# uwoseis/zephyr

Hardware: NVIDIA B200
Metric: source-frequency wavefields/sec (higher is better)
Workload: dtype c128

## Files before the change

### zephyr_b200/csrc/hz_api.cu

```cuda
#include <algorithm>
#include <cmath>
#include <cstdio>
#include <cstring>
#include <new>
#include <string>
#include <type_traits>
#include <vector>

#include "hz_platform.h"
#include "hz_assemble.cuh"
#include "hz_gemm.cuh"
#include "hz_factor.cuh"
#include "hz_factor_f32.cuh"
#include "hz_c64.cuh"
#include "hz_tf32.cuh"
#include "hz_solve.cuh"
#include "hz_survey.cuh"
#include "../../include/zephyr_b200.h"

constexpr int PROF_EVERY = 16, PROF_MAX = 4096;

struct hz_ctx {
    int device = 0, dtype = 0, disc = 0, nf = 1;
    int nx = 0, nz = 0, b = 0, nPML = 10;
// ... 4 lines not shown
    cudaStream_t stream = nullptr, stream2 = nullptr;
    cudaStream_t stream1 = nullptr;
    cudaEvent_t ev_fork = nullptr, ev_join = nullptr, ev_join0 = nullptr;
    cplx* c = nullptr;
    double *rho = nullptr, *theta = nullptr, *eps = nullptr, *delta = nullptr;
    cplx* coef = nullptr;
    cplx* Kp = nullptr;
    double* binv = nullptr;
    cplx* pmltab = nullptr;
    bool have_model = false, assembled = false, factored = false;
    cplx* Sinv = nullptr;
    cplxf* Sinv64 = nullptr;
    cplxf* Scratch64[2] = {nullptr, nullptr};
    cplxf *Rf[2] = {nullptr, nullptr}, *Cf[2] = {nullptr, nullptr}, *Pgf[2] = {nullptr, nullptr};
    int c64_tf32 = 1;
    int tf32_sms = 0;
    bool tf32_active = false;
    int ldb64 = 0;
    i64 y_S = -1;
#ifndef HZ_EMU
    alignas(64) CUtensorMap mapA;
    alignas(64) CUtensorMap mapY[2];
#endif
    int c64_fp64_factor = 1;
    cplx* Ring[2][2] = {{nullptr, nullptr}, {nullptr, nullptr}};
    i64 mid = -1;
    int store_every = 1;
    int store_used = 1;
    i64 nslots = 0;
    cplx *Rbuf[2] = {nullptr, nullptr}, *Cbuf[2] = {nullptr, nullptr};
    cplx* Pg[2] = {nullptr, nullptr};
    int* d_flag = nullptr;
    int gj_seq = 0;
    int gj_service = 2;
    int gj_colper = 1;
    int gj_coltile = 0;
    int service_fallbacks = 0;
    bool svc_on[2] = {false, false};
    cudaStream_t svc_stream[2] = {nullptr, nullptr};
    cudaEvent_t ev_svc[2] = {nullptr, nullptr};
    GjJob* d_mail = nullptr;
    GjBlockJob* d_mail2 = nullptr;
    cplx* d_Tg = nullptr;
    int* d_cflag = nullptr;
    int* d_mail_flag = nullptr;
    unsigned long long* d_done = nullptr;
    unsigned long long done_total[2] = {0, 0};
    int seq_chain[2] = {0, 0};
    cplx* Scratch[2] = {nullptr, nullptr};
    int* d_sync[2] = {nullptr, nullptr};
    size_t sync_bytes = 0;
    int gj_lean = 0;
    int gemm_3m = 1;
    int gj_colpair = 0;
    int gj_colslow = 0;
    int gj_crit = 1;
    int gj_pdl = 0;
    int gj_order = 0;
    int gj_inv = -1;
    int gj_tile = 3;
    int gj_trace = 0;
    long long* d_trace[2] = {nullptr, nullptr};
    bool trace_now = false;
    int trace_chain = 0;
    int trace_steps = 0, trace_grid = 0;
    int factor_graph = 0;
#ifndef HZ_EMU
    cudaGraphExec_t fgraph = nullptr;
#endif
    unsigned long long fgraph_key = 0, fgraph_seen = 0, fgraph_want = 0;
    long long fgraph_launches = 0;
    int fgraph_replays = 0;
    unsigned opt_epoch = 0;
    cudaEvent_t ev_svc_join[2] = {nullptr, nullptr};
    cudaEvent_t ev_fork2 = nullptr;
    int gj_mode = 1;
    cplx* Ybuf[2] = {nullptr, nullptr};
    i64 ycap = 0;
    cplx *Qsave = nullptr, *Rres = nullptr;
    i64 qcap = 0;
    int probe_check = 1;
    double probe_limit = 0.0;
    bool probe_pending = false;
    cplx* Qprobe = nullptr;
    double last_probe = -1.0;
    int* d_err = nullptr;
    double* d_norm = nullptr;
    bool prof_on = false;
    long long prof_tick[2] = {0, 0};
    std::vector<cudaEvent_t> prof_ev[2];
    long long prof_launches[2] = {0, 0};
    std::string err;
};

static void prof_begin(hz_ctx* h, int kind, cudaStream_t st, bool& armed) {
    armed = false;
    if (!h->prof_on) return;
    ++h->prof_launches[kind];
    if ((h->prof_tick[kind]++ % PROF_EVERY) != 0 || (int)h->prof_ev[kind].size() >= 2 * PROF_MAX) return;
    cudaEvent_t e0, e1;
    if (cudaEventCreate(&e0) != cudaSuccess) return;
    if (cudaEventCreate(&e1) != cudaSuccess) { cudaEventDestroy(e0); return; }
    h->prof_ev[kind].push_back(e0);
    h->prof_ev[kind].push_back(e1);
    cudaEventRecord(e0, st);
    armed = true;
// ... 757 lines not shown
    } else {
        if ((rc = launch_schur<cplx>(h, i, Xa, Xb, slot, st))) return rc;
        rc = launch_invert_v1(h, slot, chain, st);
    }
    if (rc) return rc;
    if (h->dtype == HZ_C64) {
#ifndef HZ_EMU
        if (h->tf32_active)
            HZ_LAUNCH_EW(convert_planar_kernel, dim3(blocks_for(nb2, 256)), dim3(256), 0, st, (const cplx*)slot, (float*)block64(h, i), h->b, h->ldb64);
        else
#endif
        HZ_LAUNCH_EW(convert_c64_kernel, dim3(blocks_for(nb2, 256)), dim3(256), 0, st, (const cplx*)slot, block64(h, i), nb2);
        HZ_CHECK_LAUNCH(h);
    }
    return HZ_OK;
}

static bool pair_mode(const hz_ctx* h) {
    return h->gj_mode == 4 && !(h->dtype == HZ_C64 && !h->c64_fp64_factor) && !h->gj_trace && h->gj_tile == 3 && h->gj_service != 1 && !h->gj_pdl &&
           !h->gj_coltile && h->gj_colper <= 1 && !h->gj_order && h->gj_inv < 0;
}
static int factor_pair(hz_ctx* h, i64 i0, i64 ia0, i64 ib0, int chain0, i64 i1, i64 ia1, i64 ib1, int chain1, cudaStream_t st) {
    const i64 nb2 = (i64)h->b * h->b;
    int rc;
    cplx* slot[2] = {nullptr, nullptr};
    const i64 ii[2] = {i0, i1}, ia[2] = {ia0, ia1}, ib[2] = {ib0, ib1};
    const int ch[2] = {chain0, chain1};
    for (int c = 0; c < 2; ++c) {
        if (ii[c] < 0) continue;
        const cplx* Xa = ia[c] >= 0 ? block128(h, ia[c], 0) : nullptr;
        const cplx* Xb = ib[c] >= 0 ? block128(h, ib[c], 1) : nullptr;
        slot[c] = block128(h, ii[c], ch[c]);
        cplx* start = gj_start_buffer(h) ? h->Scratch[ch[c]] : slot[c];
        if ((rc = launch_schur<cplx>(h, ii[c], Xa, Xb, start, st))) return rc;
    }
    if ((rc = launch_invert_pair(h, slot[0], ch[0], slot[1], ch[1], st))) return rc;
    if (h->dtype == HZ_C64)
        for (int c = 0; c < 2; ++c) {
            if (ii[c] < 0) continue;
#ifndef HZ_EMU
            if (h->tf32_active)
                HZ_LAUNCH_EW(convert_planar_kernel, dim3(blocks_for(nb2, 256)), dim3(256), 0, st, (const cplx*)slot[c], (float*)block64(h, ii[c]), h->b, h->ldb64);
            else
#endif
            HZ_LAUNCH_EW(convert_c64_kernel, dim3(blocks_for(nb2, 256)), dim3(256), 0, st, (const cplx*)slot[c], block64(h, ii[c]), nb2);
            HZ_CHECK_LAUNCH(h);
        }
    return HZ_OK;
}

int hz_set_option(hz_handle_t h, const char* key, double value) {
    if (!h || !key) return fail(h, HZ_EINVAL, "hz_set_option: NULL argument");
    if (!strcmp(key, "store_every") && (int)value == h->store_every) return HZ_OK;
    if (strcmp(key, "probe_check") && strcmp(key, "probe_limit") && strcmp(key, "gj_trace_chain") && strcmp(key, "factor_graph")) ++h->opt_epoch;
    if (!strcmp(key, "factor_graph")) { h->factor_graph = (int)value; return HZ_OK; }
    if (!strcmp(key, "gj_mode")) { h->gj_mode = (int)value; return HZ_OK; }
    if (!strcmp(key, "gj_colslow")) { h->gj_colslow = (int)value; return HZ_OK; }
    if (!strcmp(key, "gj_colpair")) { h->gj_colpair = (int)value; return HZ_OK; }
    if (!strcmp(key, "gj_lean")) { h->gj_lean = (int)value; return HZ_OK; }
    if (!strcmp(key, "gemm_3m")) { h->gemm_3m = (int)value; h->factored = false; return HZ_OK; }
    if (!strcmp(key, "gj_trace")) { h->gj_trace = (int)value; return HZ_OK; }
    if (!strcmp(key, "gj_trace_chain")) { h->trace_chain = (int)value; return HZ_OK; }
    if (!strcmp(key, "gj_crit")) { h->gj_crit = (int)value; return HZ_OK; }
    if (!strcmp(key, "gj_pdl")) { h->gj_pdl = (int)value; return HZ_OK; }
    if (!strcmp(key, "gj_tile")) { h->gj_tile = (int)value; return HZ_OK; }
    if (!strcmp(key, "gj_colper")) { h->gj_colper = (int)value; return HZ_OK; }
    if (!strcmp(key, "gj_coltile")) { h->gj_coltile = (int)value; return HZ_OK; }
    if (!strcmp(key, "gj_service")) { h->gj_service = (int)value; return HZ_OK; }
    if (!strcmp(key, "gj_order")) { h->gj_order = (int)value; return HZ_OK; }
    if (!strcmp(key, "gj_inv")) { h->gj_inv = (int)value; return HZ_OK; }
    if (!strcmp(key, "store_every")) {
        if (value < 1 || value > 64) return fail(h, HZ_EINVAL, "hz_set_option: store_every must be in [1, 64]");
        if ((int)value != h->store_every) h->factored = false;
        h->store_every = (int)value;
        return HZ_OK;
    }
    if (!strcmp(key, "probe_check")) { h->probe_check = (int)value; return HZ_OK; }
    if (!strcmp(key, "probe_limit")) { h->probe_limit = value; return HZ_OK; }
    if (!strcmp(key, "gj_newton")) {
        const int v = (int)value;
#ifdef HZ_EMU
        hz_gj_newton = v;
#else
        HZ_CUDA(h, cudaSetDevice(h->device));
        HZ_CUDA(h, cudaMemcpyToSymbol(hz_gj_newton, &v, sizeof(int)));
#endif
        h->factored = false;
        return HZ_OK;
    }
    if (!strcmp(key, "tf32_sms")) { h->tf32_sms = (int)value; return HZ_OK; }
    if (!strcmp(key, "c64_tf32")) { h->c64_tf32 = (int)value; h->factored = false; return HZ_OK; }
    if (!strcmp(key, "c64_fp64_factor")) { h->c64_fp64_factor = (int)value; h->factored = false; return HZ_OK; }
    return fail(h, HZ_EINVAL, std::string("hz_set_option: unknown key ") + key);
}

#ifndef HZ_EMU
template <class K>
static void preload_kernel(K kfn) {
    cudaFuncAttributes attr;
    cudaFuncGetAttributes(&attr, kfn);
}
template <class TP>
static void preload_panel_kernels() {
    preload_kernel(couple_kernel<TP, 0>); preload_kernel(residual_kernel<TP, 0>); preload_kernel(gather_col_kernel<TP>);
    preload_kernel(residual_col_kernel<TP, 0>); preload_kernel(norm2_kernel<TP>); preload_kernel(axpy_kernel<TP>);
    preload_kernel(couple_kernel<TP, 1>); preload_kernel(residual_kernel<TP, 1>); preload_kernel(residual_col_kernel<TP, 1>);
    preload_kernel(couple_kernel<TP, 2>); preload_kernel(residual_kernel<TP, 2>); preload_kernel(residual_col_kernel<TP, 2>);
    preload_kernel(finalize_kernel<TP>); preload_kernel(scatter_coo_kernel<TP>); preload_kernel(spmm_csr_kernel<TP>);
    preload_kernel(spmm_percol_kernel<TP>); preload_kernel(spmm_percol_t_kernel<TP>); preload_kernel(gradient_kernel<TP>);
    preload_kernel(misfit_kernel<TP>);
}
static void preload_factor_kernels() {
    static std::atomic<unsigned long long> done{0};
    hz_once_per_device(done, []() {
    for (const GjVariant& v : gj_variants()) {
        preload_kernel(v.fn);
        if (v.fn_lean) preload_kernel(v.fn_lean);
    }
    preload_kernel(gj_block_kernel<4, 2, 2, 4, 1, 2, 1, 2>);
    preload_kernel(gj_pair_kernel<4, 2, 2, 4, 1, 2, 1, 2>);
    preload_kernel(schur_form_kernel<cplx>);
    preload_kernel(schur_form_kernel<cplxf>);
    preload_kernel(convert_c64_kernel); preload_kernel(convert_c128_kernel);
    preload_kernel(convert_planar_kernel); preload_kernel(unconvert_planar_kernel); preload_kernel(couple_planar_kernel);
    preload_kernel(cgemm_tf32_kernel<32>); preload_kernel(cgemm_tf32_kernel<64>); preload_kernel(cgemm_tf32_kernel<128>);
    preload_kernel(cgemm_f32_kernel); preload_kernel(gj_step_f32_kernel); preload_kernel(gj_panel_kernel);
    preload_kernel(gj_step2_kernel<4, 2, 2, 4, 3>);
    preload_kernel(gj_post_quit_kernel);
    preload_kernel(gj_inverter_service);
    preload_kernel(gj_inverter_service2);
    preload_kernel(gj_post_quit2_kernel);
    preload_kernel(node_terms_kernel); preload_kernel(assemble_mz_kernel); preload_kernel(eurus_pml_tables_kernel); preload_kernel(assemble_eurus_kernel);
    preload_kernel(nearest_index_kernel); preload_kernel(kaiser_taps_kernel);
    preload_panel_kernels<cplx>();
    preload_panel_kernels<cplxf>();
    zgemm_for_each_instance<0>([](auto kfn) { preload_kernel(kfn); });
    zgemm_for_each_instance<1>([](auto kfn) { preload_kernel(kfn); });
    zgemm_for_each_instance<2>([](auto kfn) { preload_kernel(kfn); });
    cudaFuncSetAttribute(gj_inverter_service, cudaFuncAttributeMaxDynamicSharedMemorySize, GJ_SERVICE_SMEM);
    cudaFuncSetAttribute(gj_inverter_service2, cudaFuncAttributeMaxDynamicSharedMemorySize, GJ_SERVICE_SMEM);
    cudaGetLastError();
    });
}
#endif

static int factor_attempt(hz_ctx* h, int64_t twist, int* herr_out) {
    if (!h) return fail(h, HZ_EINVAL, "hz_factor: NULL handle");
    if (!h->assembled) return fail(h, HZ_ESTATE, "hz_factor: call hz_assemble first");
    HZ_CUDA(h, cudaSetDevice(h->device));
    const int nz = h->nz, b = h->b;
    i64 mid = twist < 0 ? nz / 2 : twist;
    if (mid >= nz) mid = nz - 1;
    const size_t blk = (size_t)b * b * sizeof(cplx);
    const int kst = h->store_every < 1 ? 1 : h->store_every;
    const i64 nslots = slots_needed(nz, mid, kst);
    if ((h->Sinv || h->Sinv64) && nslots != h->nslots) {
        HZ_CUDA(h, cudaStreamSynchronize(h->stream));
        HZ_CUDA(h, cudaStreamSynchronize(h->stream1));
        HZ_CUDA(h, cudaStreamSynchronize(h->stream2));
        free_dev(h->Sinv);
        free_dev(h->Sinv64);
    }
    bool want_tf32 = false;
// ... 261 lines not shown
    if (herr == 2) return fail(h, HZ_ECUDA, "hz_factor: the pivot-block inverter service did not answer (device-side wait timed out)");
    if (herr) return fail(h, HZ_ESINGULAR, "hz_factor: zero or non-finite pivot in a diagonal block (singular operator or NaN in the model)");
    h->factored = true;
    h->probe_pending = true;
    return HZ_OK;
}

int hz_factor(hz_handle_t h, int64_t twist) {
    int herr = 0;
    int rc = factor_attempt(h, twist, &herr);
    if (rc == HZ_ECUDA && herr == 2 && h && h->gj_service) {
        h->service_fallbacks += 1;
        const int fails = ++g_service_failures;
        const int saved = g_service_unavailable.exchange(1);
        if (fails == 1) fprintf(stderr, "zephyr_b200: pivot-block inverter service did not answer; this factorisation is redone with the in-kernel inverter\n");
        rc = factor_attempt(h, twist, &herr);
        if (fails < 2 && !saved) g_service_unavailable.store(0);
        else if (fails == 2) fprintf(stderr, "zephyr_b200: pivot-block inverter service failed twice in a row; using the in-kernel inverter in this process\n");
    } else if (rc == HZ_OK && h && h->gj_service && !g_service_unavailable.load()) {
        g_service_failures.store(0);
    }
    return rc;
}

int hz_get_block_inverse(hz_handle_t h, int64_t iz, void* out_host) {
    if (!h || !out_host) return fail(h, HZ_EINVAL, "hz_get_block_inverse: NULL argument");
    if (!h->factored) return fail(h, HZ_ESTATE, "hz_get_block_inverse: no factors");
    if (iz < 0 || iz >= h->nz) return fail(h, HZ_EINVAL, "hz_get_block_inverse: iz out of range");
    if (!is_stored(h, iz)) return fail(h, HZ_ESTATE, "hz_get_block_inverse: this block is not kept (store_every > 1); only checkpoints are");
    HZ_CUDA(h, cudaSetDevice(h->device));
    const i64 nb2 = (i64)h->b * h->b;
    if (h->dtype == HZ_C64 && h->tf32_active) {
        std::vector<float> tmp((size_t)2 * h->b * h->ldb64);
        HZ_CUDA(h, cudaMemcpyAsync(tmp.data(), block64(h, iz), tmp.size() * sizeof(float), cudaMemcpyDeviceToHost, h->stream));
        HZ_CUDA(h, cudaStreamSynchronize(h->stream));
        float* o = (float*)out_host;
        const size_t plane = (size_t)h->b * h->ldb64;
        for (int r = 0; r < h->b; ++r)
            for (int c = 0; c < h->b; ++c) {
                o[2 * ((size_t)r * h->b + c)] = tmp[(size_t)r * h->ldb64 + c];
                o[2 * ((size_t)r * h->b + c) + 1] = tmp[plane + (size_t)r * h->ldb64 + c];
            }
        return HZ_OK;
    }
    if (h->dtype == HZ_C64)
        HZ_CUDA(h, cudaMemcpyAsync(out_host, block64(h, iz), (size_t)nb2 * sizeof(cplxf), cudaMemcpyDeviceToHost, h->stream));
    else
        HZ_CUDA(h, cudaMemcpyAsync(out_host, h->Sinv + slot_of(h, iz) * nb2, (size_t)nb2 * sizeof(cplx), cudaMemcpyDeviceToHost, h->stream));
    HZ_CUDA(h, cudaStreamSynchronize(h->stream));
    return HZ_OK;
}

template <class TP>
static int launch_couple(hz_ctx* h, i64 i, TP* X, i64 S, TP* Y, int use_self, double lo, double hi, cudaStream_t st, int zero_self, int op) {
    const int threads = S >= 128 ? 128 : (S >= 64 ? 64 : 32);
    dim3 grid((unsigned)((S + threads - 1) / threads), h->b, 1);
#ifndef HZ_EMU
    if (std::is_same<TP, cplxf>::value && h->tf32_active) {
        const i64 ldk = h->ldb64;
        ++g_hz_launches;
        cudaLaunchConfig_t cfg = {};
        cfg.gridDim = dim3((unsigned)((S + 31) / 32), (unsigned)((h->b + 31) / 32), 1); cfg.blockDim = dim3(256); cfg.dynamicSmemBytes = 0; cfg.stream = st;
        cudaLaunchAttribute at[1];
        at[0].id = cudaLaunchAttributeProgrammaticStreamSerialization;
        at[0].val.programmaticStreamSerializationAllowed = 1;
        cfg.attrs = at; cfg.numAttrs = 1;
        cudaLaunchKernelEx(&cfg, couple_planar_kernel, (const cplx*)h->coef, h->nf, h->nx, h->nz, (int)i, (cplxf*)X, S, (float*)Y, ldk, (i64)S * ldk,
                           use_self, lo, hi, zero_self);
        HZ_CHECK_LAUNCH(h);
        return HZ_OK;
    }
#endif
    auto kfn = op == HZ_OP_T ? couple_kernel<TP, 1> : (op == HZ_OP_H ? couple_kernel<TP, 2> : couple_kernel<TP, 0>);
    HZ_LAUNCH_EW(kfn, grid, dim3(threads), 0, st, (const cplx*)h->coef, h->nf, h->nx, h->nz, (int)i, X, S, Y, use_self, lo, hi);
    HZ_CHECK_LAUNCH(h);
    return HZ_OK;
}

static int launch_block_gemm(hz_ctx* h, i64 i, const cplx* Y, cplx* X, i64 S, double alpha, int beta, cudaStream_t st, int op) {
    GemmParams p;
    p.A = h->Sinv + slot_of(h, i) * (i64)h->b * h->b; p.lda = h->b;
    p.B = Y; p.ldb = S;
    p.C = X + i * (i64)h->nx * S; p.ldc = S;
    p.M = h->b; p.N = (int)S; p.K = h->b;
    p.alpha = alpha; p.beta = beta;
    p.sub_c0 = p.sub_c1 = 0;
    p.row_nx = h->nf > 1 ? h->nx : 0;
    p.row_fs = h->N;
    bool armed;
    prof_begin(h, 0, st, armed);
    const bool m3 = (h->gemm_3m & 1) != 0;
    if (op == HZ_OP_T) zgemm_launch<1>(p, st, h->num_sms, -1, m3);
    else if (op == HZ_OP_H) zgemm_launch<2>(p, st, h->num_sms, -1, m3);
    else zgemm_launch<0>(p, st, h->num_sms, -1, m3);
    prof_end(h, 0, st, armed);
    HZ_CHECK_LAUNCH(h);
    return HZ_OK;
}
static int launch_block_gemm(hz_ctx* h, i64 i, const cplxf* Y, cplxf* X, i64 S, double alpha, int beta, cudaStream_t st, int ) {
#ifndef HZ_EMU
    if (h->tf32_active) {
        Tf32Params tp;
        tp.M = h->b; tp.N = (int)S; tp.K = h->b;
        tp.a_plane0 = (int)(2 * slot_of(h, i));
        tp.y_plane0 = 0;
        tp.C = X + i * (i64)h->nx * S; tp.ldc = S;
        tp.alpha = (float)alpha;
        tp.row_nx = h->nf > 1 ? h->nx : 0;
        tp.row_fs = h->N;
        tp.k_per_split = 0;
        tp.dbg = nullptr; tp.mode = 0; tp.force_split = 0;
        bool armed;
        prof_begin(h, 0, st, armed);
        cgemm_tf32_launch(h->mapA, h->mapY[(const cplx*)Y == h->Ybuf[1] ? 1 : 0], tp, h->tf32_sms > 0 ? h->tf32_sms : h->num_sms, st);
        prof_end(h, 0, st, armed);
        HZ_CHECK_LAUNCH(h);
        return HZ_OK;
    }
#endif
    CGemmParams p;
    p.A = block64(h, i); p.lda = h->b;
    p.B = Y; p.ldb = S;
    p.C = X + i * (i64)h->nx * S; p.ldc = S;
    p.M = h->b; p.N = (int)S; p.K = h->b;
    p.alpha = (float)alpha; p.beta = beta;
    p.row_nx = h->nf > 1 ? h->nx : 0;
    p.row_fs = h->N;
    bool armed;
    prof_begin(h, 0, st, armed);
    cgemm_f32_launch(p, st);
    prof_end(h, 0, st, armed);
    HZ_CHECK_LAUNCH(h);
    return HZ_OK;
}

static int recompute_segment(hz_ctx* h, int chain, i64 j, cudaStream_t st) {
    const int k = h->store_used;
    const i64 len = chain == 0 ? h->mid : (i64)h->nz - 1 - h->mid;
    const i64 p0 = j * k, p1 = std::min<i64>((j + 1) * k - 1, len - 1);
    const i64 nb2 = (i64)h->b * h->b;
    for (i64 p = p0; p < p1; ++p) {
        const i64 i = chain_row(h, chain, p), prev = p > 0 ? chain_row(h, chain, p - 1) : -1;
        if (h->dtype == HZ_C64 && h->c64_fp64_factor && p == p0 && prev >= 0) {
#ifndef HZ_EMU
            if (h->tf32_active)
                HZ_LAUNCH_EW(unconvert_planar_kernel, dim3(blocks_for(nb2, 256)), dim3(256), 0, st, (const float*)block64(h, prev), h->Ring[chain][prev & 1], h->b, h->ldb64);
            else
#endif
            HZ_LAUNCH_EW(convert_c128_kernel, dim3(blocks_for(nb2, 256)), dim3(256), 0, st, (const cplxf*)block64(h, prev), h->Ring[chain][prev & 1], nb2);
            HZ_CHECK_LAUNCH(h);
        }
        const int rc = factor_block(h, i, chain == 0 ? prev : -1, chain == 1 ? prev : -1, chain, st);
        if (rc) return rc;
    }
    return HZ_OK;
}

template <class TP>
static int solve_inplace(hz_ctx* h, TP* X, i64 S, i64 zf, i64 zl, int op) {
    const i64 nz = h->nz, mid = h->mid;
    const int k = h->store_used;
    if (zf < 0 || zf >= nz) zf = 0;
    if (zl < 0 || zl >= nz) zl = nz - 1;
    if (zl < zf) { zf = 0; zl = nz - 1; }
    cudaStream_t st[2] = {h->stream, h->stream2};
    TP* Y[2] = {(TP*)h->Ybuf[0], (TP*)h->Ybuf[1]};
    const i64 len[2] = {mid, nz - 1 - mid};
    int rc;
    HZ_CUDA(h, cudaEventRecord(h->ev_fork, st[0]));
    HZ_CUDA(h, cudaStreamWaitEvent(st[1], h->ev_fork, 0));
    const bool top_fwd = zf < mid, bot_fwd = zl > mid;
    const i64 pfirst[2] = {zf, nz - 1 - zl};
    for (int c = 0; c < 2; ++c) {
        for (i64 p = pfirst[c]; p < len[c]; ++p) {
            if (k > 1 && (p == pfirst[c] || p % k == 0) && (rc = recompute_segment(h, c, p / k, st[c]))) return rc;
            const i64 i = chain_row(h, c, p);
            const double sg = p > pfirst[c] ? -1.0 : 0.0;
            if ((rc = launch_couple<TP>(h, i, X, S, Y[c], 1, c == 0 ? sg : 0.0, c == 0 ? 0.0 : sg, st[c], 1, op))) return rc;
            if ((rc = launch_block_gemm(h, i, (const TP*)Y[c], X, S, 1.0, 0, st[c], op))) return rc;
        }
    }
    HZ_CUDA(h, cudaEventRecord(h->ev_join, st[1]));
    HZ_CUDA(h, cudaStreamWaitEvent(st[0], h->ev_join, 0));
    if ((rc = launch_couple<TP>(h, mid, X, S, Y[0], 1, top_fwd ? -1.0 : 0.0, bot_fwd ? -1.0 : 0.0, st[0], 1, op))) return rc;
    if ((rc = launch_block_gemm(h, mid, (const TP*)Y[0], X, S, 1.0, 0, st[0], op))) return rc;
    HZ_CUDA(h, cudaEventRecord(h->ev_fork, st[0]));
    HZ_CUDA(h, cudaStreamWaitEvent(st[1], h->ev_fork, 0));
    const i64 nmax = len[0] > len[1] ? len[0] : len[1];
    for (i64 t = 1; t <= nmax; ++t) {
        for (int c = 0; c < 2; ++c) {
            if (t > len[c]) continue;
            const i64 p = len[c] - t, i = chain_row(h, c, p);
            if (k > 1 && (t == 1 || p % k == k - 1) && (rc = recompute_segment(h, c, p / k, st[c]))) return rc;
            if ((rc = launch_couple<TP>(h, i, X, S, Y[c], 0, c == 0 ? 0.0 : 1.0, c == 0 ? 1.0 : 0.0, st[c], 0, op))) return rc;
            if ((rc = launch_block_gemm(h, i, (const TP*)Y[c], X, S, -1.0, 1, st[c], op))) return rc;
        }
    }
    HZ_CUDA(h, cudaEventRecord(h->ev_join, st[1]));
    HZ_CUDA(h, cudaStreamWaitEvent(st[0], h->ev_join, 0));
    if (k > 1) {
        int herr = 0;
        HZ_CUDA(h, cudaMemcpyAsync(&herr, h->d_err, sizeof(int), cudaMemcpyDeviceToHost, st[0]));
        HZ_CUDA(h, cudaStreamSynchronize(st[0]));
        if (herr) return fail(h, HZ_ESINGULAR, "hz_solve: zero or non-finite pivot while recomputing block inverses between checkpoints");
    }
    return HZ_OK;
}

template <class TP>
static int launch_residual(hz_ctx* h, const TP* X, const TP* Q, i64 S, TP* R, int op) {
    const int threads = S >= 128 ? 128 : (S >= 64 ? 64 : 32);
    const i64 rows = (i64)h->nf * h->N;
    dim3 grid((unsigned)((S + threads - 1) / threads), (unsigned)(rows < 65535 ? rows : 65535), (unsigned)((rows + 65534) / 65535));
    auto kfn = op == HZ_OP_T ? residual_kernel<TP, 1> : (op == HZ_OP_H ? residual_kernel<TP, 2> : residual_kernel<TP, 0>);
    HZ_LAUNCH_EW(kfn, grid, dim3(threads), 0, h->stream, (const cplx*)h->coef, h->nf, h->nx, h->nz, X, Q, S, R);
    HZ_CHECK_LAUNCH(h);
    return HZ_OK;
}

template <class TP>
static int solve_impl(hz_ctx* h, int op, TP* X, int64_t S, double premul_re, double premul_im, int conjugate,
                      int64_t z_first, int64_t z_last, int refine, double* resid_host) {
    const i64 rows = (i64)h->nf * h->N, n = rows * S;
    if (h->ycap < S) {
        HZ_CUDA(h, cudaStreamSynchronize(h->stream));
        HZ_CUDA(h, cudaStreamSynchronize(h->stream2));
        for (int k = 0; k < 2; ++k) {
            free_dev(h->Ybuf[k]);
            HZ_CUDA(h, cudaMalloc((void**)&h->Ybuf[k], (size_t)h->b * S * sizeof(cplx)));
        }
        h->ycap = S;
        h->y_S = -1;
    }
#ifndef HZ_EMU
    if (std::is_same<TP, cplxf>::value && h->tf32_active && h->y_S != S) {
        for (int k = 0; k < 2; ++k)
            if (!t32_make_map(&h->mapY[k], (const float*)h->Ybuf[k], h->b, S, 2, h->ldb64, T32_KS, t32_tile_n(S), false))
                return fail(h, HZ_ECUDA, "hz_solve: cuTensorMapEncodeTiled failed for the right-hand-side planes");
        h->y_S = S;
    }
#endif
    const bool want_resid = refine > 0 || resid_host != nullptr;
    if (want_resid && h->qcap < S) {
        HZ_CUDA(h, cudaStreamSynchronize(h->stream));
        free_dev(h->Qsave); free_dev(h->Rres);
        HZ_CUDA(h, cudaMalloc((void**)&h->Qsave, (size_t)n * sizeof(TP)));
        HZ_CUDA(h, cudaMalloc((void**)&h->Rres, (size_t)n * sizeof(TP)));
        h->qcap = S;
// ... 367 lines not shown
```

### zephyr_b200/csrc/hz_gemm.cuh

```cuda
#pragma once
#include "hz_platform.h"

struct GemmParams {
    const cplx* A; i64 lda;
    const cplx* B; i64 ldb;
    cplx* C; i64 ldc;
    int M, N, K;
    double alpha;
    int beta;
    int sub_c0, sub_c1;
    int row_nx; i64 row_fs;
};

constexpr int GEMM_KB = 32;
constexpr int GEMM_LDA = GEMM_KB + 4;

template <int MI, int NI, int WM, int WN, int STAGES, int KS = 1>
struct GemmCfg {
    static constexpr int TM = 8 * MI * WM, TN = 8 * NI * WN, THREADS = 32 * WM * WN * KS;
    static constexpr int LDB = TN + 2;
    static constexpr int A_ELEMS = TM * GEMM_LDA, B_ELEMS = GEMM_KB * LDB;
    static constexpr int SMEM = STAGES * (A_ELEMS + B_ELEMS) * (int)sizeof(cplx);
};

template <int MI, int NI, int WM, int WN, int STAGES, int KS = 1, bool M3 = false, int OPA = 0>
__global__ void __launch_bounds__(32 * WM * WN * KS, 1) zgemm_dmma_kernel(GemmParams p) {
    typedef GemmCfg<MI, NI, WM, WN, STAGES, KS> Cfg;
    constexpr int TM = Cfg::TM, TN = Cfg::TN, NT = Cfg::THREADS, LDB = Cfg::LDB;
    constexpr bool AT = OPA != 0, ACONJ = OPA == 2;
    constexpr int LDAT = TM + 2;
    static_assert(OPA >= 0 && OPA <= 2, "op(A) is N, T or C");
    static_assert(!AT || GEMM_KB * LDAT <= Cfg::A_ELEMS, "the k-major A tile must fit the A stage");
    HZ_SMEM(smem_raw);
    cplx* sA = reinterpret_cast<cplx*>(smem_raw);
    cplx* sB = sA + STAGES * Cfg::A_ELEMS;

    const int tid = threadIdx.x;
    const int warp = tid >> 5, lane = tid & 31;
    const int g = lane >> 2, t = lane & 3;
    const int wk = warp / (WM * WN), w2 = warp % (WM * WN);
    const int wm = w2 / WN, wn = w2 % WN;
    const int m0 = blockIdx.y * TM, n0 = blockIdx.x * TN;
    const int KT = (p.K + GEMM_KB - 1) / GEMM_KB;

    static_assert(NT % GEMM_KB == 0 && NT % TN == 0, "staging assumes whole rows per thread stride");
    constexpr int RA = AT ? NT / TM : NT / GEMM_KB, RB = NT / TN;
    constexpr int NA = AT ? (GEMM_KB + RA - 1) / RA : (TM * GEMM_KB + NT - 1) / NT, NBL = (GEMM_KB * TN + NT - 1) / NT;
    const int a_r0 = AT ? tid / TM : tid / GEMM_KB, a_kk = AT ? tid % TM : tid % GEMM_KB;
    const int b_k0 = tid / TN, b_c = tid % TN;
    const cplx* a_base = AT ? p.A + (i64)a_r0 * p.lda + (m0 + a_kk) : p.A + (i64)(m0 + a_r0) * p.lda + a_kk;
    const cplx* b_base = p.B + (i64)b_k0 * p.ldb + (n0 + b_c);
    const i64 a_step = (i64)RA * p.lda, b_step = (i64)RB * p.ldb;
    const bool a_col_ok = AT && a_r0 < RA && m0 + a_kk < p.M;
    const bool b_col_ok = n0 + b_c < p.N;
    auto stage_op = [&](int op, int k0, cplx* a, cplx* b) {
        if (op < NA) {
            const int u = op, r = a_r0 + u * RA;
            if constexpr (AT) {
                if (a_r0 < RA && r < GEMM_KB) {
                    const bool ok = a_col_ok && (k0 + r < p.K);
                    cp_async16(a + r * LDAT + a_kk, ok ? a_base + (i64)k0 * p.lda + u * a_step : p.A, ok);
                }
            } else if (u * NT + tid < TM * GEMM_KB) {
                const bool ok = (m0 + r < p.M) && (k0 + a_kk < p.K);
                cp_async16(a + r * GEMM_LDA + a_kk, ok ? a_base + u * a_step + k0 : p.A, ok);
            }
        } else {
            const int u = op - NA, kk = b_k0 + u * RB;
            if (u * NT + tid < GEMM_KB * TN) {
                const bool ok = b_col_ok && (k0 + kk < p.K);
                cp_async16(b + kk * LDB + b_c, ok ? b_base + (i64)k0 * p.ldb + u * b_step : p.B, ok);
            }
        }
    };
    auto load_stage = [&](int kt, int st) {
#pragma unroll
        for (int op = 0; op < NA + NBL; ++op) stage_op(op, kt * GEMM_KB, sA + st * Cfg::A_ELEMS, sB + st * Cfg::B_ELEMS);
    };

    double cre[MI][NI][2], cim[MI][NI][2];
    double c2[M3 ? MI : 1][M3 ? NI : 1][2];
#pragma unroll
    for (int mi = 0; mi < MI; ++mi)
#pragma unroll
        for (int ni = 0; ni < NI; ++ni) {
            cre[mi][ni][0] = cre[mi][ni][1] = cim[mi][ni][0] = cim[mi][ni][1] = 0.0;
            if constexpr (M3) c2[mi][ni][0] = c2[mi][ni][1] = 0.0;
        }

#pragma unroll
    for (int s = 0; s < STAGES - 1; ++s) {
        if (s < KT) load_stage(s, s);
        cp_async_commit();
    }

    constexpr int S4 = GEMM_KB / 4 / KS;
    constexpr int OPS = (NA + NBL + S4 - 1) / S4;
    for (int kt = 0; kt < KT; ++kt) {
        cp_async_wait<STAGES - 2>();
        __syncthreads();
        const int nk = kt + STAGES - 1;
        const bool refill = nk < KT;
        cplx* na = sA + (nk % STAGES) * Cfg::A_ELEMS;
        cplx* nb = sB + (nk % STAGES) * Cfg::B_ELEMS;
        const cplx* a = AT ? sA + (kt % STAGES) * Cfg::A_ELEMS + t * LDAT + wm * MI * 8 + g
                           : sA + (kt % STAGES) * Cfg::A_ELEMS + (wm * MI * 8 + g) * GEMM_LDA + t;
        const cplx* b = sB + (kt % STAGES) * Cfg::B_ELEMS + t * LDB + wn * NI * 8 + g;
#pragma unroll
        for (int k4s = 0; k4s < S4; ++k4s) {
            const int k4 = k4s * KS + wk;
            cplx af[MI], bf[NI];
#pragma unroll
            for (int mi = 0; mi < MI; ++mi) af[mi] = AT ? a[k4 * 4 * LDAT + mi * 8] : a[mi * 8 * GEMM_LDA + k4 * 4];
#pragma unroll
            for (int ni = 0; ni < NI; ++ni) bf[ni] = b[k4 * 4 * LDB + ni * 8];
            if constexpr (M3) {
                double as[MI], bs[NI];
#pragma unroll
                for (int mi = 0; mi < MI; ++mi) as[mi] = ACONJ ? af[mi].re - af[mi].im : af[mi].re + af[mi].im;
#pragma unroll
                for (int ni = 0; ni < NI; ++ni) bs[ni] = bf[ni].re + bf[ni].im;
#pragma unroll
                for (int mi = 0; mi < MI; ++mi)
#pragma unroll
                    for (int ni = 0; ni < NI; ++ni) {
                        dmma884(cre[mi][ni][0], cre[mi][ni][1], af[mi].re, bf[ni].re);
                        dmma884(c2[mi][ni][0], c2[mi][ni][1], af[mi].im, bf[ni].im);
                    }
                if (refill) {
#pragma unroll
                    for (int op = k4s * OPS; op < (k4s + 1) * OPS && op < NA + NBL; ++op) stage_op(op, nk * GEMM_KB, na, nb);
                }
#pragma unroll
                for (int mi = 0; mi < MI; ++mi)
#pragma unroll
                    for (int ni = 0; ni < NI; ++ni) dmma884(cim[mi][ni][0], cim[mi][ni][1], as[mi], bs[ni]);
            } else {
#pragma unroll
            for (int mi = 0; mi < MI; ++mi)
#pragma unroll
                for (int ni = 0; ni < NI; ++ni) {
                    dmma884(cre[mi][ni][0], cre[mi][ni][1], af[mi].re, bf[ni].re);
                    dmma884(cim[mi][ni][0], cim[mi][ni][1], af[mi].re, bf[ni].im);
                }
            if (refill) {
// ... 34 lines not shown
            for (int mi = 0; mi < MI; ++mi)
#pragma unroll
                for (int ni = 0; ni < NI; ++ni) {
                    red[(mi * NI + ni) * 64] = mk(cre[mi][ni][0], cim[mi][ni][0]);
                    red[(mi * NI + ni) * 64 + 1] = mk(cre[mi][ni][1], cim[mi][ni][1]);
                }
        }
        __syncthreads();
        if (wk > 0) return;
#pragma unroll
        for (int mi = 0; mi < MI; ++mi)
#pragma unroll
            for (int ni = 0; ni < NI; ++ni)
#pragma unroll
                for (int j = 0; j < 2; ++j) {
                    const cplx v = red[(mi * NI + ni) * 64 + j];
                    cre[mi][ni][j] += v.re;
                    cim[mi][ni][j] += v.im;
                }
    }

#pragma unroll
    for (int mi = 0; mi < MI; ++mi) {
        const int r = m0 + (wm * MI + mi) * 8 + g;
        if (r >= p.M) continue;
        const i64 crow = p.row_nx ? (i64)(r / p.row_nx) * p.row_fs + (r % p.row_nx) : (i64)r;
        cplx* crp = p.C + crow * p.ldc;
#pragma unroll
        for (int ni = 0; ni < NI; ++ni) {
#pragma unroll
            for (int j = 0; j < 2; ++j) {
                const int cidx = n0 + (wn * NI + ni) * 8 + 2 * t + j;
                if (cidx >= p.N) continue;
                cplx v = mk(p.alpha * cre[mi][ni][j], p.alpha * cim[mi][ni][j]);
                if (p.beta) {
                    cplx cin;
                    if (cidx >= p.sub_c0 && cidx < p.sub_c1) cin = mk(r == cidx ? 1.0 : 0.0);
                    else cin = crp[cidx];
                    v = v + cin;
                }
                crp[cidx] = v;
            }
        }
    }
}

template <int MI, int NI, int WM, int WN, int STAGES, int KS = 1, bool M3 = false, int OPA = 0>
static inline int zgemm_launch_cfg(const GemmParams& p, cudaStream_t stream) {
    typedef GemmCfg<MI, NI, WM, WN, STAGES, KS> Cfg;
    auto kfn = zgemm_dmma_kernel<MI, NI, WM, WN, STAGES, KS, M3, OPA>;
    static std::atomic<unsigned long long> configured{0};
    hz_once_per_device(configured, [&]() { cudaFuncSetAttribute(kfn, cudaFuncAttributeMaxDynamicSharedMemorySize, Cfg::SMEM); });
    dim3 grid((p.N + Cfg::TN - 1) / Cfg::TN, (p.M + Cfg::TM - 1) / Cfg::TM, 1);
    HZ_LAUNCH_IND(kfn, grid, dim3(Cfg::THREADS), Cfg::SMEM, stream, p);
    return 0;
}

struct GemmTile { int tm, tn; };
static const GemmTile kGemmTiles[] = {{64, 64}, {56, 64}, {48, 64}, {40, 64}, {32, 64}, {32, 32}, {16, 32}};
constexpr int kNumGemmTiles = sizeof(kGemmTiles) / sizeof(kGemmTiles[0]);

static inline int zgemm_pick(int M, int N, int num_sms) {
    double best = -1.0;
    int besti = 0;
    for (int i = 0; i < kNumGemmTiles; ++i) {
        const i64 tiles = (i64)((M + kGemmTiles[i].tm - 1) / kGemmTiles[i].tm) * ((N + kGemmTiles[i].tn - 1) / kGemmTiles[i].tn);
        const i64 waves = (tiles + num_sms - 1) / num_sms;
        double eff = (double)M * N / ((double)waves * num_sms * kGemmTiles[i].tm * kGemmTiles[i].tn);
        eff *= 1.0 + 0.02 * (kGemmTiles[i].tm * kGemmTiles[i].tn) / 4096.0;
        if (eff > best) { best = eff; besti = i; }
    }
    return besti;
}

static inline int zgemm_tile_id(int cand, bool m3) {
    const int which = cand + (m3 ? 16 : 0);
    return which == 17 ? 24 : which;
}

template <int OPA, class F>
static inline void zgemm_for_each_instance(F f) {
    f(zgemm_dmma_kernel<4, 2, 2, 4, 3, 1, false, OPA>); f(zgemm_dmma_kernel<7, 1, 1, 8, 3, 1, false, OPA>);
    f(zgemm_dmma_kernel<6, 1, 1, 8, 3, 1, false, OPA>); f(zgemm_dmma_kernel<5, 1, 1, 8, 3, 1, false, OPA>);
    f(zgemm_dmma_kernel<2, 2, 2, 4, 4, 1, false, OPA>); f(zgemm_dmma_kernel<2, 1, 2, 4, 4, 1, false, OPA>);
    f(zgemm_dmma_kernel<1, 1, 2, 4, 4, 1, false, OPA>);
    f(zgemm_dmma_kernel<4, 2, 2, 4, 3, 1, true, OPA>); f(zgemm_dmma_kernel<6, 1, 1, 8, 3, 1, true, OPA>);
    f(zgemm_dmma_kernel<5, 1, 1, 8, 3, 1, true, OPA>); f(zgemm_dmma_kernel<2, 2, 2, 4, 4, 1, true, OPA>);
    f(zgemm_dmma_kernel<2, 1, 2, 4, 4, 1, true, OPA>); f(zgemm_dmma_kernel<1, 1, 2, 4, 4, 1, true, OPA>);
    f(zgemm_dmma_kernel<7, 2, 1, 4, 3, 2, true, OPA>);
    if constexpr (OPA == 0) {
        f(zgemm_dmma_kernel<7, 1, 1, 8, 3, 2>); f(zgemm_dmma_kernel<4, 2, 2, 4, 3, 2>); f(zgemm_dmma_kernel<6, 1, 1, 8, 3, 2>);
        f(zgemm_dmma_kernel<5, 1, 1, 8, 3, 2>); f(zgemm_dmma_kernel<7, 2, 1, 4, 3>); f(zgemm_dmma_kernel<7, 2, 1, 4, 3, 2>);
        f(zgemm_dmma_kernel<7, 1, 1, 8, 3, 1, true>); f(zgemm_dmma_kernel<7, 2, 1, 4, 3, 1, true>); f(zgemm_dmma_kernel<7, 1, 1, 8, 3, 2, true>);
    }
}

template <int OPA = 0>
static inline int zgemm_launch(const GemmParams& p, cudaStream_t stream, int num_sms, int force_tile = -1, bool m3 = false) {
    const int which = force_tile >= 0 ? force_tile : zgemm_tile_id(zgemm_pick(p.M, p.N, num_sms), m3);
    switch (which) {
        case 16: return zgemm_launch_cfg<4, 2, 2, 4, 3, 1, true, OPA>(p, stream);
        case 18: return zgemm_launch_cfg<6, 1, 1, 8, 3, 1, true, OPA>(p, stream);
        case 19: return zgemm_launch_cfg<5, 1, 1, 8, 3, 1, true, OPA>(p, stream);
        case 20: return zgemm_launch_cfg<2, 2, 2, 4, 4, 1, true, OPA>(p, stream);
        case 21: return zgemm_launch_cfg<2, 1, 2, 4, 4, 1, true, OPA>(p, stream);
        case 22: return zgemm_launch_cfg<1, 1, 2, 4, 4, 1, true, OPA>(p, stream);
        case 24: return zgemm_launch_cfg<7, 2, 1, 4, 3, 2, true, OPA>(p, stream);
// ... 26 lines not shown
```

### zephyr_b200/csrc/hz_solve.cuh

```cuda
#pragma once
#include "hz_platform.h"
#include "hz_factor.cuh"
#include "hz_c64.cuh"

template <int OP>
__device__ __forceinline__ cplx op_coef(const cplx* __restrict__ coef, int nf, int fr, int fc, int slot, i64 node, i64 nbr, i64 N) {
    if constexpr (OP == 0) return coef_plane(coef, nf, fr, fc, slot, N)[node];
    const cplx v = coef_plane(coef, nf, fc, fr, 8 - slot, N)[nbr];
    return OP == 2 ? cconj(v) : v;
}

template <class TP, int OP = 0>
__global__ void couple_kernel(const cplx* __restrict__ coef, int nf, int nx, int nz, int i,
                              const TP* __restrict__ X, i64 S, TP* __restrict__ Y,
                              int use_self, double sgn_lo, double sgn_hi) {
    const i64 s = (i64)blockIdx.x * blockDim.x + threadIdx.x;
    const int rl = blockIdx.y;
    if (s >= S) return;
    const i64 N = (i64)nx * nz;
    const int fr = rl / nx, ix = rl % nx;
    const i64 node = (i64)i * nx + ix;
    cplx acc = mk(0.0);
    if (use_self) acc = ldp(&X[((i64)fr * N + node) * S + s]);
    for (int side = 0; side < 2; ++side) {
        const double sg = side == 0 ? sgn_lo : sgn_hi;
        if (sg == 0.0) continue;
        const int dzs = side == 0 ? -1 : 1;
        cplx part = mk(0.0);
        for (int fc = 0; fc < nf; ++fc) {
#pragma unroll
            for (int a = -1; a <= 1; ++a) {
                if (ix + a < 0 || ix + a >= nx) continue;
                const i64 nbr = (i64)(i + dzs) * nx + ix + a;
                const cplx cf = op_coef<OP>(coef, nf, fr, fc, (dzs + 1) * 3 + a + 1, node, nbr, N);
                cfma(part, cf, ldp(&X[((i64)fc * N + nbr) * S + s]));
            }
        }
        acc = acc + sg * part;
    }
    stp(&Y[(i64)rl * S + s], acc);
}

template <class TP, int OP = 0>
__global__ void residual_kernel(const cplx* __restrict__ coef, int nf, int nx, int nz,
                                const TP* __restrict__ X, const TP* __restrict__ Q, i64 S,
                                TP* __restrict__ R) {
    const i64 s = (i64)blockIdx.x * blockDim.x + threadIdx.x;
    if (s >= S) return;
    const i64 N = (i64)nx * nz;
    const i64 row = (i64)blockIdx.y + (i64)blockIdx.z * 65535;
    if (row >= (i64)nf * N) return;
    const int fr = (int)(row / N);
    const i64 node = row % N;
    const int iz = (int)(node / nx), ix = (int)(node % nx);
    cplx acc = ldp(&Q[row * S + s]);
    for (int fc = 0; fc < nf; ++fc)
#pragma unroll
        for (int dzs = -1; dzs <= 1; ++dzs) {
            if (iz + dzs < 0 || iz + dzs >= nz) continue;
#pragma unroll
            for (int a = -1; a <= 1; ++a) {
                if (ix + a < 0 || ix + a >= nx) continue;
                const i64 nbr = node + (i64)dzs * nx + a;
                const cplx cf = op_coef<OP>(coef, nf, fr, fc, (dzs + 1) * 3 + a + 1, node, nbr, N);
                const cplx xv = ldp(&X[((i64)fc * N + nbr) * S + s]);
                acc = acc - cf * xv;
            }
        }
    stp(&R[row * S + s], acc);
}

template <class TP>
__global__ void gather_col_kernel(const TP* __restrict__ X, i64 S, i64 col, i64 rows, cplx* __restrict__ out) {
    for (i64 r = (i64)blockIdx.x * blockDim.x + threadIdx.x; r < rows; r += (i64)gridDim.x * blockDim.x) out[r] = ldp(&X[r * S + col]);
}
template <class TP, int OP = 0>
__global__ void residual_col_kernel(const cplx* __restrict__ coef, int nf, int nx, int nz, const TP* __restrict__ X, i64 S, i64 col,
                                    const cplx* __restrict__ q, double* __restrict__ out) {
    const i64 N = (i64)nx * nz, rows = (i64)nf * N;
    double sr = 0.0, sq = 0.0;
    for (i64 row = (i64)blockIdx.x * blockDim.x + threadIdx.x; row < rows; row += (i64)gridDim.x * blockDim.x) {
        const int fr = (int)(row / N);
        const i64 node = row % N;
        const int iz = (int)(node / nx), ix = (int)(node % nx);
        const cplx qv = q[row];
        cplx acc = qv;
        for (int fc = 0; fc < nf; ++fc)
#pragma unroll
            for (int dzs = -1; dzs <= 1; ++dzs) {
                if (iz + dzs < 0 || iz + dzs >= nz) continue;
#pragma unroll
                for (int a = -1; a <= 1; ++a) {
                    if (ix + a < 0 || ix + a >= nx) continue;
                    const i64 nbr = node + (i64)dzs * nx + a;
                    const cplx cf = op_coef<OP>(coef, nf, fr, fc, (dzs + 1) * 3 + a + 1, node, nbr, N);
// ... 62 lines not shown
```

Baseline: 322.2.

## Add strip-tiled coupling kernel and PDL chaining across block-sweep launches

Adds a new coupling kernel that tiles several rows per thread and shares neighbour X loads in registers. Coefficients go into shared memory, and the kernel is used by default for c128 sweeps. The coupling and block GEMM kernels are now launched with programmatic dependent launch. Each one preloads its independent data (coefficients, A tiles) before waiting on the previous kernel, which is meant to hide launch gaps and prologue latency in the long serial chain. The risk is extra correctness exposure around PDL ordering, and higher register use from the per-thread windows.

```diff
diff --git a/zephyr_b200/csrc/hz_api.cu b/zephyr_b200/csrc/hz_api.cu
--- a/zephyr_b200/csrc/hz_api.cu
+++ b/zephyr_b200/csrc/hz_api.cu
@@ -80,6 +80,7 @@
     size_t sync_bytes = 0;
     int gj_lean = 0;
     int gemm_3m = 1;
+    int sweep_chain = 1;
     int gj_colpair = 0;
     int gj_colslow = 0;
     int gj_crit = 1;
@@ -943,7 +944,9 @@
 int hz_set_option(hz_handle_t h, const char* key, double value) {
     if (!h || !key) return fail(h, HZ_EINVAL, "hz_set_option: NULL argument");
     if (!strcmp(key, "store_every") && (int)value == h->store_every) return HZ_OK;
-    if (strcmp(key, "probe_check") && strcmp(key, "probe_limit") && strcmp(key, "gj_trace_chain") && strcmp(key, "factor_graph")) ++h->opt_epoch;
+    if (strcmp(key, "probe_check") && strcmp(key, "probe_limit") && strcmp(key, "gj_trace_chain") && strcmp(key, "factor_graph") &&
+        strcmp(key, "sweep_chain")) ++h->opt_epoch;
+    if (!strcmp(key, "sweep_chain")) { h->sweep_chain = (int)value; return HZ_OK; }
     if (!strcmp(key, "factor_graph")) { h->factor_graph = (int)value; return HZ_OK; }
     if (!strcmp(key, "gj_mode")) { h->gj_mode = (int)value; return HZ_OK; }
     if (!strcmp(key, "gj_colslow")) { h->gj_colslow = (int)value; return HZ_OK; }
@@ -1000,6 +1003,10 @@
     preload_kernel(finalize_kernel<TP>); preload_kernel(scatter_coo_kernel<TP>); preload_kernel(spmm_csr_kernel<TP>);
     preload_kernel(spmm_percol_kernel<TP>); preload_kernel(spmm_percol_t_kernel<TP>); preload_kernel(gradient_kernel<TP>);
     preload_kernel(misfit_kernel<TP>);
+    if constexpr (std::is_same<TP, cplx>::value) {
+        preload_kernel(couple_strip_kernel<0, 1>); preload_kernel(couple_strip_kernel<1, 1>); preload_kernel(couple_strip_kernel<2, 1>);
+        preload_kernel(couple_strip_kernel<0, 2>); preload_kernel(couple_strip_kernel<1, 2>); preload_kernel(couple_strip_kernel<2, 2>);
+    }
 }
 static void preload_factor_kernels() {
     static std::atomic<unsigned long long> done{0};
@@ -1367,7 +1374,7 @@
 }
 
 template <class TP>
-static int launch_couple(hz_ctx* h, i64 i, TP* X, i64 S, TP* Y, int use_self, double lo, double hi, cudaStream_t st, int zero_self, int op) {
+static int launch_couple(hz_ctx* h, i64 i, TP* X, i64 S, TP* Y, int use_self, double lo, double hi, cudaStream_t st, int zero_self, int op, int chain) {
     const int threads = S >= 128 ? 128 : (S >= 64 ? 64 : 32);
     dim3 grid((unsigned)((S + threads - 1) / threads), h->b, 1);
 #ifndef HZ_EMU
@@ -1386,13 +1393,31 @@
         return HZ_OK;
     }
 #endif
+    if constexpr (std::is_same<TP, cplx>::value) {
+        if (chain) {
+            CoupleParams p;
+            p.coef = h->coef; p.nf = h->nf; p.nx = h->nx; p.nz = h->nz; p.i = (int)i;
+            p.X = X; p.S = S; p.Y = Y;
+            p.use_self = use_self; p.sgn_lo = lo; p.sgn_hi = hi;
+            p.pdl = chain == 2;
+            const dim3 sgrid((unsigned)((S + COUPLE_SPAN - 1) / COUPLE_SPAN), (unsigned)((h->nx + COUPLE_ROWS - 1) / COUPLE_ROWS), (unsigned)h->nf);
+            const dim3 block(COUPLE_SPAN, COUPLE_RG);
+            const int smem = h->nf > 1 ? couple_strip_smem<2>() : couple_strip_smem<1>();
+            auto kfn = h->nf > 1 ? (op == HZ_OP_T ? couple_strip_kernel<1, 2> : (op == HZ_OP_H ? couple_strip_kernel<2, 2> : couple_strip_kernel<0, 2>))
+                                 : (op == HZ_OP_T ? couple_strip_kernel<1, 1> : (op == HZ_OP_H ? couple_strip_kernel<2, 1> : couple_strip_kernel<0, 1>));
+            if (p.pdl) HZ_LAUNCH_PDL(kfn, sgrid, block, smem, st, p);
+            else HZ_LAUNCH(kfn, sgrid, block, smem, st, p);
+            HZ_CHECK_LAUNCH(h);
+            return HZ_OK;
+        }
+    }
     auto kfn = op == HZ_OP_T ? couple_kernel<TP, 1> : (op == HZ_OP_H ? couple_kernel<TP, 2> : couple_kernel<TP, 0>);
     HZ_LAUNCH_EW(kfn, grid, dim3(threads), 0, st, (const cplx*)h->coef, h->nf, h->nx, h->nz, (int)i, X, S, Y, use_self, lo, hi);
     HZ_CHECK_LAUNCH(h);
     return HZ_OK;
 }
 
-static int launch_block_gemm(hz_ctx* h, i64 i, const cplx* Y, cplx* X, i64 S, double alpha, int beta, cudaStream_t st, int op) {
+static int launch_block_gemm(hz_ctx* h, i64 i, const cplx* Y, cplx* X, i64 S, double alpha, int beta, cudaStream_t st, int op, bool pdl) {
     GemmParams p;
     p.A = h->Sinv + slot_of(h, i) * (i64)h->b * h->b; p.lda = h->b;
     p.B = Y; p.ldb = S;
@@ -1404,6 +1429,7 @@
     p.row_fs = h->N;
     bool armed;
     prof_begin(h, 0, st, armed);
+    p.pdl = pdl && !armed;
     const bool m3 = (h->gemm_3m & 1) != 0;
     if (op == HZ_OP_T) zgemm_launch<1>(p, st, h->num_sms, -1, m3);
     else if (op == HZ_OP_H) zgemm_launch<2>(p, st, h->num_sms, -1, m3);
@@ -1412,7 +1438,7 @@
     HZ_CHECK_LAUNCH(h);
     return HZ_OK;
 }
-static int launch_block_gemm(hz_ctx* h, i64 i, const cplxf* Y, cplxf* X, i64 S, double alpha, int beta, cudaStream_t st, int ) {
+static int launch_block_gemm(hz_ctx* h, i64 i, const cplxf* Y, cplxf* X, i64 S, double alpha, int beta, cudaStream_t st, int , bool ) {
 #ifndef HZ_EMU
     if (h->tf32_active) {
         Tf32Params tp;
@@ -1482,23 +1508,26 @@
     TP* Y[2] = {(TP*)h->Ybuf[0], (TP*)h->Ybuf[1]};
     const i64 len[2] = {mid, nz - 1 - mid};
     int rc;
+    const bool chain = h->sweep_chain && std::is_same<TP, cplx>::value;
+    auto cmode = [&](bool after_gemm) { return chain ? (after_gemm ? 2 : 1) : 0; };
     HZ_CUDA(h, cudaEventRecord(h->ev_fork, st[0]));
     HZ_CUDA(h, cudaStreamWaitEvent(st[1], h->ev_fork, 0));
     const bool top_fwd = zf < mid, bot_fwd = zl > mid;
     const i64 pfirst[2] = {zf, nz - 1 - zl};
     for (int c = 0; c < 2; ++c) {
         for (i64 p = pfirst[c]; p < len[c]; ++p) {
-            if (k > 1 && (p == pfirst[c] || p % k == 0) && (rc = recompute_segment(h, c, p / k, st[c]))) return rc;
+            const bool recomp = k > 1 && (p == pfirst[c] || p % k == 0);
+            if (recomp && (rc = recompute_segment(h, c, p / k, st[c]))) return rc;
             const i64 i = chain_row(h, c, p);
             const double sg = p > pfirst[c] ? -1.0 : 0.0;
-            if ((rc = launch_couple<TP>(h, i, X, S, Y[c], 1, c == 0 ? sg : 0.0, c == 0 ? 0.0 : sg, st[c], 1, op))) return rc;
-            if ((rc = launch_block_gemm(h, i, (const TP*)Y[c], X, S, 1.0, 0, st[c], op))) return rc;
+            if ((rc = launch_couple<TP>(h, i, X, S, Y[c], 1, c == 0 ? sg : 0.0, c == 0 ? 0.0 : sg, st[c], 1, op, cmode(p > pfirst[c] && !recomp)))) return rc;
+            if ((rc = launch_block_gemm(h, i, (const TP*)Y[c], X, S, 1.0, 0, st[c], op, chain))) return rc;
         }
     }
     HZ_CUDA(h, cudaEventRecord(h->ev_join, st[1]));
     HZ_CUDA(h, cudaStreamWaitEvent(st[0], h->ev_join, 0));
-    if ((rc = launch_couple<TP>(h, mid, X, S, Y[0], 1, top_fwd ? -1.0 : 0.0, bot_fwd ? -1.0 : 0.0, st[0], 1, op))) return rc;
-    if ((rc = launch_block_gemm(h, mid, (const TP*)Y[0], X, S, 1.0, 0, st[0], op))) return rc;
+    if ((rc = launch_couple<TP>(h, mid, X, S, Y[0], 1, top_fwd ? -1.0 : 0.0, bot_fwd ? -1.0 : 0.0, st[0], 1, op, cmode(false)))) return rc;
+    if ((rc = launch_block_gemm(h, mid, (const TP*)Y[0], X, S, 1.0, 0, st[0], op, chain))) return rc;
     HZ_CUDA(h, cudaEventRecord(h->ev_fork, st[0]));
     HZ_CUDA(h, cudaStreamWaitEvent(st[1], h->ev_fork, 0));
     const i64 nmax = len[0] > len[1] ? len[0] : len[1];
@@ -1506,9 +1535,10 @@
         for (int c = 0; c < 2; ++c) {
             if (t > len[c]) continue;
             const i64 p = len[c] - t, i = chain_row(h, c, p);
-            if (k > 1 && (t == 1 || p % k == k - 1) && (rc = recompute_segment(h, c, p / k, st[c]))) return rc;
-            if ((rc = launch_couple<TP>(h, i, X, S, Y[c], 0, c == 0 ? 0.0 : 1.0, c == 0 ? 1.0 : 0.0, st[c], 0, op))) return rc;
-            if ((rc = launch_block_gemm(h, i, (const TP*)Y[c], X, S, -1.0, 1, st[c], op))) return rc;
+            const bool recomp = k > 1 && (t == 1 || p % k == k - 1);
+            if (recomp && (rc = recompute_segment(h, c, p / k, st[c]))) return rc;
+            if ((rc = launch_couple<TP>(h, i, X, S, Y[c], 0, c == 0 ? 0.0 : 1.0, c == 0 ? 1.0 : 0.0, st[c], 0, op, cmode(t > 1 && !recomp)))) return rc;
+            if ((rc = launch_block_gemm(h, i, (const TP*)Y[c], X, S, -1.0, 1, st[c], op, chain))) return rc;
         }
     }
     HZ_CUDA(h, cudaEventRecord(h->ev_join, st[1]));
diff --git a/zephyr_b200/csrc/hz_gemm.cuh b/zephyr_b200/csrc/hz_gemm.cuh
--- a/zephyr_b200/csrc/hz_gemm.cuh
+++ b/zephyr_b200/csrc/hz_gemm.cuh
@@ -10,6 +10,7 @@
     int beta;
     int sub_c0, sub_c1;
     int row_nx; i64 row_fs;
+    int pdl = 0;
 };
 
 constexpr int GEMM_KB = 32;
@@ -73,10 +74,6 @@
             }
         }
     };
-    auto load_stage = [&](int kt, int st) {
-#pragma unroll
-        for (int op = 0; op < NA + NBL; ++op) stage_op(op, kt * GEMM_KB, sA + st * Cfg::A_ELEMS, sB + st * Cfg::B_ELEMS);
-    };
 
     double cre[MI][NI][2], cim[MI][NI][2];
     double c2[M3 ? MI : 1][M3 ? NI : 1][2];
@@ -90,7 +87,21 @@
 
 #pragma unroll
     for (int s = 0; s < STAGES - 1; ++s) {
-        if (s < KT) load_stage(s, s);
+        if (s < KT) {
+#pragma unroll
+            for (int op = 0; op < NA; ++op) stage_op(op, s * GEMM_KB, sA + s * Cfg::A_ELEMS, sB + s * Cfg::B_ELEMS);
+        }
+    }
+    if (p.pdl) {
+        hz_grid_launch_dependents();
+        hz_grid_dependency_wait();
+    }
+#pragma unroll
+    for (int s = 0; s < STAGES - 1; ++s) {
+        if (s < KT) {
+#pragma unroll
+            for (int op = NA; op < NA + NBL; ++op) stage_op(op, s * GEMM_KB, sA + s * Cfg::A_ELEMS, sB + s * Cfg::B_ELEMS);
+        }
         cp_async_commit();
     }
 
@@ -231,7 +242,8 @@
     static std::atomic<unsigned long long> configured{0};
     hz_once_per_device(configured, [&]() { cudaFuncSetAttribute(kfn, cudaFuncAttributeMaxDynamicSharedMemorySize, Cfg::SMEM); });
     dim3 grid((p.N + Cfg::TN - 1) / Cfg::TN, (p.M + Cfg::TM - 1) / Cfg::TM, 1);
-    HZ_LAUNCH_IND(kfn, grid, dim3(Cfg::THREADS), Cfg::SMEM, stream, p);
+    if (p.pdl) HZ_LAUNCH_PDL(kfn, grid, dim3(Cfg::THREADS), Cfg::SMEM, stream, p);
+    else HZ_LAUNCH_IND(kfn, grid, dim3(Cfg::THREADS), Cfg::SMEM, stream, p);
     return 0;
 }
 
diff --git a/zephyr_b200/csrc/hz_solve.cuh b/zephyr_b200/csrc/hz_solve.cuh
--- a/zephyr_b200/csrc/hz_solve.cuh
+++ b/zephyr_b200/csrc/hz_solve.cuh
@@ -41,6 +41,81 @@
     stp(&Y[(i64)rl * S + s], acc);
 }
 
+constexpr int COUPLE_SPAN = 32, COUPLE_RG = 8, COUPLE_R = 4, COUPLE_ROWS = COUPLE_RG * COUPLE_R;
+
+struct CoupleParams {
+    const cplx* coef; int nf, nx, nz, i;
+    const cplx* X; i64 S; cplx* Y;
+    int use_self; double sgn_lo, sgn_hi;
+    int pdl;
+};
+
+template <int NF>
+constexpr int couple_strip_smem() { return COUPLE_ROWS * 2 * NF * 3 * (int)sizeof(cplx); }
+
+template <int OP, int NF>
+__global__ void __launch_bounds__(COUPLE_SPAN * COUPLE_RG) couple_strip_kernel(CoupleParams p) {
+    HZ_SMEM(smem_raw);
+    cplx* cs = reinterpret_cast<cplx*>(smem_raw);
+    const int tx = threadIdx.x, ty = threadIdx.y, tid = ty * COUPLE_SPAN + tx;
+    const int fr = blockIdx.z, ix0 = blockIdx.y * COUPLE_ROWS;
+    const int nx = p.nx;
+    const i64 N = (i64)nx * p.nz, S = p.S;
+    const bool act[2] = {p.sgn_lo != 0.0, p.sgn_hi != 0.0};
+    for (int e = tid; e < COUPLE_ROWS * 2 * NF * 3; e += COUPLE_SPAN * COUPLE_RG) {
+        const int a = e % 3 - 1, fc = (e / 3) % NF, side = (e / (3 * NF)) % 2, ix = ix0 + e / (6 * NF);
+        const int dzs = side == 0 ? -1 : 1;
+        if (act[side] && ix < nx && ix + a >= 0 && ix + a < nx)
+            cs[e] = op_coef<OP == 2 ? 1 : OP>(p.coef, NF, fr, fc, (dzs + 1) * 3 + a + 1, (i64)p.i * nx + ix, (i64)(p.i + dzs) * nx + ix + a, N);
+    }
+    if (p.pdl) {
+        hz_grid_launch_dependents();
+        hz_grid_dependency_wait();
+    }
+    __syncthreads();
+    const i64 s = (i64)blockIdx.x * COUPLE_SPAN + tx;
+    const int r0 = ty * COUPLE_R, ixb = ix0 + r0;
+    if (s >= S || ixb >= nx) return;
+    cplx xw[2][NF][COUPLE_R + 2], xself[COUPLE_R];
+#pragma unroll
+    for (int side = 0; side < 2; ++side) {
+        if (!act[side]) continue;
+        const cplx* xr = p.X + ((i64)(p.i + (side == 0 ? -1 : 1)) * nx + ixb - 1) * S + s;
+#pragma unroll
+        for (int fc = 0; fc < NF; ++fc)
+#pragma unroll
+            for (int k = 0; k < COUPLE_R + 2; ++k)
+                xw[side][fc][k] = (ixb - 1 + k >= 0 && ixb - 1 + k < nx) ? ldp(xr + ((i64)fc * N + k) * S) : mk(0.0);
+    }
+#pragma unroll
+    for (int j = 0; j < COUPLE_R; ++j)
+        xself[j] = (p.use_self && ixb + j < nx) ? ldp(p.X + ((i64)fr * N + (i64)p.i * nx + ixb + j) * S + s) : mk(0.0);
+#pragma unroll
+    for (int j = 0; j < COUPLE_R; ++j) {
+        const int ix = ixb + j;
+        if (ix >= nx) break;
+        cplx acc = mk(0.0);
+        if (p.use_self) acc = xself[j];
+#pragma unroll
+        for (int side = 0; side < 2; ++side) {
+            const double sg = side == 0 ? p.sgn_lo : p.sgn_hi;
+            if (sg == 0.0) continue;
+            const cplx* c = cs + ((r0 + j) * 2 + side) * NF * 3;
+            cplx part = mk(0.0);
+#pragma unroll
+            for (int fc = 0; fc < NF; ++fc) {
+#pragma unroll
+                for (int a = -1; a <= 1; ++a) {
+                    if (ix + a < 0 || ix + a >= nx) continue;
+                    cfma(part, OP == 2 ? cconj(c[fc * 3 + a + 1]) : c[fc * 3 + a + 1], xw[side][fc][j + a + 1]);
+                }
+            }
+            acc = acc + sg * part;
+        }
+        stp(p.Y + ((i64)fr * nx + ix) * S + s, acc);
+    }
+}
+
 template <class TP, int OP = 0>
 __global__ void residual_kernel(const cplx* __restrict__ coef, int nf, int nx, int nz,
                                 const TP* __restrict__ X, const TP* __restrict__ Q, i64 S,
```

Result: no change. 323.2 (median of 6 runs) (+0.3%).
